# apache/cassandra

Hardware: NVIDIA H100
Metric: compaction MB/s (uncompressed in) (higher is better)
Workload: dtype u8

## Files before the change

cassandra_b200/csrc/compact.cu:

```cuda
#include "engine.cuh"
#include "scan.cuh"
#include "codec_defs.cuh"
#include "partition.cuh"
#include "partition_tile.cuh"
#include "meta.cuh"
#include "index_walk.cuh"
#include <climits>
#include <vector>
#include <algorithm>
#include <cmath>

using namespace b200c;

namespace b200c {

int compress_stream_device(b200c_ctx* c, int comp, const uint8_t* d_in, uint64_t n, int chunk_len, int max_clen,
                           uint8_t* d_out, uint64_t out_cap, uint64_t* d_offs, uint64_t* out_len, uint32_t* digest, int ws_base);
int compress_slots_device(b200c_ctx* c, int comp, const uint8_t* d_in, uint64_t n, int chunk_len, int max_clen,
                          uint8_t* slots, int stride, uint32_t* file_len, uint32_t* seg_raw);
int pack_digest_device(b200c_ctx* c, const uint8_t* slots, int stride, const uint32_t* file_len, const uint32_t* seg_raw, uint64_t nchunks,
                       uint8_t* d_out, uint64_t out_cap, uint64_t* d_offs, uint64_t* out_len, uint32_t* digest, int ws_base);
int decompress_stream_device(b200c_ctx* c, int comp, const uint8_t* d_data, uint64_t data_len, const uint64_t* d_offs, uint64_t nchunks,
                             int chunk_len, int max_clen, uint64_t data_length, uint8_t* d_out, int verify, ChunkErr* d_err, uint64_t chunk0, uint64_t count, int tag,
                             const uint8_t* tail, uint64_t tail_off);
int decompress_multi_device(b200c_ctx* c, K1Seg* segs, int nseg, int verify, ChunkErr* d_err, int ws_slot);
int raw_chunks_device(b200c_ctx* c, bool ingest, const RawArgs& a);
int raw_stream_device(b200c_ctx* c, const uint8_t* d_in, uint64_t n, int chunk_len, uint8_t* d_out, uint64_t* d_crc, uint32_t* digest, int ws_base);

enum { IB = 256 };
static_assert(IW_PAD <= 64, "the Index.db workspace keeps 64 bytes behind every input (index_walk.cuh)");
#ifndef B200C_K4_STAGED_DEFAULT
#define B200C_K4_STAGED_DEFAULT 0
#endif
#ifndef B200C_K1_BATCH_DEFAULT
#define B200C_K1_BATCH_DEFAULT true
#endif
#define NONE64 (~0ull)

enum { WS_U = 16, WS_CD, WS_CO, WS_IDX, WS_PARAMS, WS_BBASE, WS_ISTART, WS_ICNT, WS_IEND, WS_IHIT, WS_IBAD, WS_ISCAN,
// ... 511 lines not shown
    return ((uint64_t)fanin_class(m, bound, wide_bound) * ntiles + (j >> tile_shift)) * SORT_BINS + (m - 1) * SORT_BUCKETS + bucket;
}
__global__ void __launch_bounds__(256) k_class_hist(const uint64_t* __restrict__ op_first, const uint64_t* __restrict__ bound, uint64_t nparts,
                                                    uint32_t tile_shift, uint64_t ntiles, uint64_t wide_bound, unsigned long long* __restrict__ hist) {
    for (uint64_t j = (uint64_t)blockIdx.x * blockDim.x + threadIdx.x; j < nparts; j += (uint64_t)gridDim.x * blockDim.x)
        atomicAdd(&hist[sort_key((uint32_t)(op_first[j + 1] - op_first[j]), bound[j], j, tile_shift, ntiles, wide_bound)], 1ull);
}
__global__ void __launch_bounds__(256) k_fanin_scatter(const uint64_t* __restrict__ op_first, const uint64_t* __restrict__ bound, uint64_t nparts,
                                                       uint32_t tile_shift, uint64_t ntiles, uint64_t wide_bound, unsigned long long* __restrict__ cursor, uint32_t* __restrict__ list) {
    uint64_t j = (uint64_t)blockIdx.x * blockDim.x + threadIdx.x;
    bool valid = j < nparts;
    uint64_t key = valid ? sort_key((uint32_t)(op_first[j + 1] - op_first[j]), bound[j], j, tile_shift, ntiles, wide_bound) : ~0ull;
    uint32_t peers = __match_any_sync(FULL_MASK, key);
    int lane = threadIdx.x & 31, leader = __ffs(peers) - 1;
    unsigned long long base = 0;
    if (valid && lane == leader) base = atomicAdd(&cursor[key], (unsigned long long)__popc(peers));
    base = __shfl_sync(FULL_MASK, base, leader);
    if (valid) list[base + __popc(peers & ((1u << lane) - 1u))] = (uint32_t)j;
}

typedef Cur32 K4Cur;
enum { SLOT_BYTES = sizeof(K4Cur), K4_SMEM_COLS = 8 };

struct K4Args {
    const CParams* P; const uint64_t* contrib; const uint64_t* op_first; const uint32_t* list; const uint64_t* upos; const uint64_t* pbase;
    const uint64_t* kp; const uint16_t* klen; const int64_t* tok;
    uint64_t* dsize; uint32_t* ipay; uint32_t* nblk; uint32_t* ihead; uint32_t* st_munf; uint32_t* st_rows; uint8_t* ovf;
    const uint64_t* doff; const uint64_t* dcapv; const uint64_t* dpos; const uint64_t* ipos; uint8_t* dbase; uint8_t* iout; DevErr* err; int mode;
    uint64_t jlo, jhi;
    const uint64_t* ioff; const uint32_t* icapv; uint8_t* iscr;
    int m3_nblk;
    const uint8_t* only_big;
    StatGlobal* sg; TdropTable* td; uint32_t* ccount;
};

template <bool EMIT> __device__ __forceinline__ bool k4_prologue(const K4Args& a, uint64_t j, uint8_t*& dout, uint64_t& dcap, uint64_t& dposv, uint8_t*& iout, uint32_t& nbf, uint32_t& ipf, uint32_t& ixs_cap) {
    dout = nullptr; dcap = ~0ull; dposv = 0; iout = nullptr; nbf = 0; ipf = 0; ixs_cap = 0;
    if (!EMIT) return true;
    if (a.mode == 1) {
        if (a.only_big && !a.only_big[j]) return false;
        dout = a.dbase + a.doff[j]; dcap = a.dcapv[j];
        uint32_t slot = a.icapv[j];
        if (slot) { iout = a.iscr + a.ioff[j]; nbf = (slot - IXS_HEAD) / IXS_BLOCK_STRIDE; ixs_cap = nbf * IXS_PER_BLOCK; }
        return true;
    }
    if (!a.dsize[j] || j < a.jlo || j >= a.jhi) return false;
    if (a.mode == 3 && !(a.ovf[j] || (a.m3_nblk && a.nblk[j] > 1))) return false;
    dout = a.dbase + a.dpos[j]; dposv = a.dpos[j]; iout = a.iout + a.ipos[j]; nbf = a.nblk[j]; ipf = a.ipay[j];
    return true;
}
template <bool EMIT> __device__ __forceinline__ void k4_epilogue(const K4Args& a, uint64_t j, uint64_t c0, PartOut out, PartStats st, int e) {
    if (EMIT && a.mode >= 2) { if (e || out.dsize != a.dsize[j]) report_err(a.err, 8, 0, j); return; }
    if (e) { uint64_t en = a.contrib[c0]; int src = (int)((en >> 56) & 0x7F); report_err(a.err, e == PERR_UNSUPPORTED ? 9 : 4, src, a.upos[a.pbase[src] + (en & 0xFFFFFFFFFFull)] - a.P->in[src].ubase); out = PartOut{0, 0, 0, 0, 0}; st = PartStats{0, 0}; }
    a.dsize[j] = out.dsize; a.ipay[j] = out.ipay; a.nblk[j] = out.nblk; a.ihead[j] = out.ihead; a.ovf[j] = (uint8_t)out.ovf;
    if (a.ccount) a.ccount[j] = out.cells;
    a.st_munf[j] = (uint32_t)st.merged_unfiltereds; a.st_rows[j] = (uint32_t)st.rows_out;
}

template <int M_CAP, int NT, bool EMIT, bool CX = false>
__global__ void __launch_bounds__(NT, 384 / NT) k_partition_thr(const K4Args a, uint64_t lo, uint64_t hi) {
    extern __shared__ __align__(16) uint8_t s_raw[];
    const int ncols_s = a.P->mcols <= K4_SMEM_COLS ? a.P->mcols : 0;
    const int stride = M_CAP * SLOT_BYTES + ncols_s * (int)sizeof(MCell) + 8;
    K4Cur* cur = (K4Cur*)(s_raw + (size_t)threadIdx.x * stride);
    MCell merged_local[MAXCOLS];
    MCell* merged = ncols_s ? (MCell*)(cur + M_CAP) : merged_local;
    DT open_dt[M_CAP];
    uint64_t t = lo + (uint64_t)blockIdx.x * NT + threadIdx.x;
    if (t >= hi) return;
    uint64_t j = a.list[t];
    uint8_t *dout, *iout; uint64_t dcap, dposv; uint32_t nbf, ipf, ixs_cap;
    if (!k4_prologue<EMIT>(a, j, dout, dcap, dposv, iout, nbf, ipf, ixs_cap)) return;
    uint64_t c0 = a.op_first[j]; uint32_t m = (uint32_t)(a.op_first[j + 1] - c0);
    PartOut out{0, 0, 0, 0, 0}; PartStats st{0, 0}; int e = 0;
    StatAcc acc; const bool stats = a.sg != nullptr && a.mode == 1;
    if (stats) acc.init(a.P->now, a.td);
    if (m > (uint32_t)M_CAP) e = PERR_UNSUPPORTED;
    else process_partition<EMIT, K4Cur, XlateGlobal, M_CAP, CX>(*a.P, XlateGlobal(), a.contrib, c0, m, a.upos, a.pbase, a.kp, a.klen, a.tok, dout, dcap, dposv, iout, nbf, ipf, ixs_cap, cur, open_dt, merged, out, st, e, stats ? &acc : nullptr);
    k4_epilogue<EMIT>(a, j, c0, out, st, e);
    if (stats && !e) stat_flush(a.sg, acc);
}

template <int S, bool EMIT>
__global__ void __launch_bounds__(128) k_partition_warp(const K4Args a, uint64_t lo, uint64_t hi) {
    extern __shared__ __align__(16) uint8_t s_raw[];
    auto tile = cg::tiled_partition<32>(cg::this_thread_block());
    const int tid = threadIdx.x / 32;
// ... 102 lines not shown
    StatAcc acc; acc.init(sP->now, a.td);
    for (uint32_t t = tid; t < np; t += ST_THREADS) {
        const uint32_t j = j0 + s_order[t];
        const uint64_t cj = a.op_first[j]; const uint32_t m = (uint32_t)(a.op_first[j + 1] - cj);
        const uint32_t m_uni = min((uint32_t)ST_MAXM, __reduce_max_sync(__activemask(), m));
        uint8_t *dout, *iout; uint64_t dcap, dposv; uint32_t nbf, ipf, ixs_cap;
        if (!k4_prologue<true>(a, j, dout, dcap, dposv, iout, nbf, ipf, ixs_cap)) continue;
        PartOut out{0, 0, 0, 0, 0}; PartStats st{0, 0}; int e = 0;
        if (m > (uint32_t)ST_MAXM || cj - c0 + m > (uint64_t)ST_CUR_CAP) e = PERR_UNSUPPORTED;
        else process_partition<true>(*sP, xl, a.contrib, cj, m, a.upos, a.pbase, a.kp, a.klen, a.tok, dout, dcap, dposv, iout, nbf, ipf, ixs_cap, curs + (cj - c0), open_dt, merged, out, st, e,
                                     a.sg ? &acc : nullptr, m_uni);
        k4_epilogue<true>(a, j, cj, out, st, e);
    }
    if (a.sg) stat_flush_warp(a.sg, acc);
}

__global__ void __launch_bounds__(256) k_bounds(const uint64_t* __restrict__ contrib, const uint64_t* __restrict__ op_first, uint64_t nparts,
                                                const uint64_t* __restrict__ upos, const uint64_t* __restrict__ pbase, uint64_t* __restrict__ bound,
                                                uint32_t column_index_size, uint32_t* __restrict__ icap, uint32_t* __restrict__ insz, uint8_t* __restrict__ big) {
    uint64_t j = (uint64_t)blockIdx.x * blockDim.x + threadIdx.x;
    if (j >= nparts) return;
    uint64_t sum = 0;
    for (uint64_t c = op_first[j]; c < op_first[j + 1]; c++) { uint64_t e = contrib[c]; uint64_t g = pbase[(e >> 56) & 0x7F] + (e & 0xFFFFFFFFFFull); sum += upos[g + 1] - upos[g]; }
    uint64_t b = (sum + (sum >> 2) + 32 + 15) & ~15ull;
    bound[j] = b;
    insz[j] = (uint32_t)min(sum, (uint64_t)0xFFFFFFFFull);
    big[j] = (sum > (uint64_t)ST_MAXP || op_first[j + 1] - op_first[j] > (uint64_t)ST_MAXM) ? 1 : 0;
    uint64_t nb_max = b / column_index_size + 2;
    icap[j] = (b > column_index_size && nb_max < (1u << 23)) ? (uint32_t)(IXS_HEAD + nb_max * IXS_BLOCK_STRIDE) : 0u;
}

__global__ void __launch_bounds__(256) k_gather(uint64_t nparts, const uint64_t* __restrict__ dsize, const uint64_t* __restrict__ dpos, const uint64_t* __restrict__ bpos,
                                                const uint8_t* __restrict__ ovf, const uint8_t* __restrict__ scratch, uint8_t* __restrict__ uout) {
    uint64_t j = (uint64_t)blockIdx.x * 8 + (threadIdx.x >> 5);
    if (j >= nparts) return;
    uint64_t n = dsize[j];
    if (!n || ovf[j]) return;
    const uint8_t* s = scratch + bpos[j]; uint8_t* d = uout + dpos[j];
    int lane = threadIdx.x & 31;
    for (uint64_t i = lane; i < n; i += 32) d[i] = s[i];
}

__global__ void __launch_bounds__(256) k_index_simple(const CParams* __restrict__ Pp, uint64_t nparts, const uint64_t* __restrict__ contrib, const uint64_t* __restrict__ op_first,
        const uint64_t* __restrict__ upos, const uint64_t* __restrict__ pbase, const uint64_t* __restrict__ dsize, const uint64_t* __restrict__ dpos,
        const uint32_t* __restrict__ nblk, const uint8_t* __restrict__ ovf, const uint32_t* __restrict__ ihead, const uint64_t* __restrict__ ipos, uint8_t* __restrict__ iout) {
    uint64_t j = (uint64_t)blockIdx.x * blockDim.x + threadIdx.x;
    if (j >= nparts || !dsize[j] || nblk[j] > 1 || ovf[j]) return;
    uint64_t e = contrib[op_first[j]]; uint64_t g = pbase[(e >> 56) & 0x7F] + (e & 0xFFFFFFFFFFull);
    const uint8_t* k = Pp->U + upos[g];
    uint32_t n = ihead[j];
    Sink<true> s{iout + ipos[j], 0, true, ~0ull};
    s.copy(k, n); s.vint(dpos[j]); s.u8(0);
}

__global__ void __launch_bounds__(128) k_index_promoted(const CParams* __restrict__ Pp, uint64_t nparts, const uint64_t* __restrict__ contrib, const uint64_t* __restrict__ op_first,
        const uint64_t* __restrict__ upos, const uint64_t* __restrict__ pbase, const uint64_t* __restrict__ dsize, const uint64_t* __restrict__ dpos,
        const uint32_t* __restrict__ nblk, const uint8_t* __restrict__ ovf, const uint32_t* __restrict__ ihead, const uint32_t* __restrict__ ipay, const uint64_t* __restrict__ ipos,
        const uint64_t* __restrict__ ioff, const uint32_t* __restrict__ icap, const uint8_t* __restrict__ iscr, uint8_t* __restrict__ iout) {
    uint64_t j = (uint64_t)blockIdx.x * blockDim.x + threadIdx.x;
    if (j >= nparts || !dsize[j] || nblk[j] <= 1 || ovf[j]) return;
    uint64_t e = contrib[op_first[j]]; uint64_t g = pbase[(e >> 56) & 0x7F] + (e & 0xFFFFFFFFFFull);
    const uint8_t* k = Pp->U + upos[g];
    const uint8_t* slot = iscr + ioff[j];
    const uint32_t nb_max = (icap[j] - IXS_HEAD) / IXS_BLOCK_STRIDE, nb = nblk[j], n = ihead[j];
    DT pd; pd.mfda = ((const int64_t*)slot)[0]; pd.ldt = ((const int64_t*)slot)[1];
    const uint32_t pdsz = dt_is_live(pd) ? 1u : 12u, hdr_len = (uint32_t)((const int64_t*)slot)[2];
    const uint32_t infos = ipay[j] - vint_size(hdr_len) - pdsz - vint_size(nb) - 4 * nb;
    Sink<true> s{iout + ipos[j], 0, true, ~0ull};
    s.copy(k, n); s.vint(dpos[j]); s.vint(ipay[j]);
    s.vint(hdr_len); write_partition_dt(s, pd); s.vint(nb);
    s.copy(slot + IXS_HEAD + 4 * (size_t)nb_max, infos); s.copy(slot + IXS_HEAD, 4 * nb);
}

// ... 63 lines not shown
template <bool WIDE> int k4_staged(b200c_ctx* c, const K4Args& ka, uint64_t ntiles, size_t smem, const uint32_t* tstart, const uint8_t* big) {
    B200C_LAUNCH(c, k_partition_staged<WIDE>, (unsigned)ntiles, ST_THREADS, smem, ka, tstart, big);
    return B200C_OK;
}
template <bool WIDE> void k4_staged_attr(size_t smem) { cudaFuncSetAttribute(k_partition_staged<WIDE>, cudaFuncAttributeMaxDynamicSharedMemorySize, (int)smem); }

struct CompactCall {
    b200c_ctx* const c; const b200c_manifest* const m; b200c_result* const res;
    const bool dev, lcs; const int K;
    const bool raw_out, to_host_stream;
    const cudaMemcpyKind in_kind;
    Pinned* const P; const cudaStream_t st, cs;
    const std::chrono::steady_clock::time_point t_start = std::chrono::steady_clock::now();
    bool want_meta = false, two_pass = false;
    int rc = B200C_OK;

    struct Need { uint64_t h2d_a, h2d_b, k1_a, k1_b; };
    bool have_summaries = true, sliced = false, deferred = false, istream = false;
    int nr = 1;
    std::vector<IdxSlice> isl;
    std::vector<int64_t> T;
    std::vector<std::vector<IdxSlice>> psl;
    std::vector<uint64_t> pustart;
    std::vector<std::vector<uint64_t>> psb;
    std::vector<Need> need;
    std::vector<uint64_t> range_bytes, range_end;
    std::vector<uint64_t> h2d_next, k1_next;
    std::vector<std::vector<uint64_t>> co_host;
    std::vector<uint64_t> ubase, ibase, cbase, obase, bbase;
    uint64_t uo = 0, io = 0, co = 0, oo = 0, in_bytes = 0, bytes_read = 0;
    CParams hp; std::vector<InDesc> hin;

    uint8_t *U = nullptr, *CD = nullptr, *IDX = nullptr; uint64_t *CO = nullptr, *d_bbase = nullptr, *d_summ = nullptr; CParams* dP = nullptr;
    DevErr* d_err = nullptr; ChunkErr* d_cerr = nullptr; RunStats* d_stats = nullptr; unsigned long long *d_hist = nullptr, *d_rbytes = nullptr;
    std::vector<const uint8_t*> k1_data, k1_tail; std::vector<const uint64_t*> k1_offs; std::vector<uint64_t> k1_tail_off; std::vector<K1Seg> segs;
    int k1_batch_env = 0;
    StatGlobal* d_sg = nullptr; TdropTable* d_td = nullptr; uint32_t* d_bloom = nullptr; uint8_t *d_mkeys = nullptr, *d_sument = nullptr; uint64_t* d_sumoff = nullptr;
    uint64_t written_total = 0, samples_total = 0, sument_bound = 0, bloom_words = 0; uint32_t meta_interval = 128;
    uint64_t total_parts = 0, slow_inputs = 0; std::vector<uint64_t> pcount, pbase;
    int64_t* d_tok = nullptr; uint64_t *d_kp = nullptr, *d_upos = nullptr, *d_pbase = nullptr, *d_pcount = nullptr, *d_range = nullptr; uint16_t* d_klen = nullptr;
    OutStream os; uint64_t L = 0;
    uint64_t ubase_total = 0, ilen_total = 0, ncontrib_total = 0, nparts_total = 0;
    uint64_t tail_len = 0; const uint8_t* tail_ptr = nullptr;
    bool index_fits = true;
    uint64_t nparts = 0, ulen_out = 0, ilen_out = 0, n_le8 = 0, n_le12 = 0, n_le16 = 0, n_le32 = 0;
    uint64_t *d_contrib = nullptr, *d_opfirst = nullptr, *d_bound = nullptr, *d_bpos = nullptr, *d_ioff = nullptr, *d_dsize = nullptr, *d_dpos = nullptr, *d_ipos = nullptr, *d_wrank = nullptr;
    uint32_t *d_list = nullptr, *d_icap = nullptr, *d_insz = nullptr, *d_ipay = nullptr, *d_nblk = nullptr, *d_ihead = nullptr, *d_isize = nullptr;
    uint32_t *d_stmunf = nullptr, *d_strows = nullptr, *d_ccount = nullptr, *d_wflag = nullptr; uint8_t *d_ovf = nullptr, *d_big = nullptr;
    uint8_t *UOUT = nullptr, *IOUT = nullptr, *ISCR = nullptr, *SCRATCH = nullptr;
    size_t smem8 = 0, smem12 = 0, smem16 = 0, smem64 = 0, cell_smem32 = 0;
    K4Args ka;
    int lcs_stride = 0; uint8_t* slots = nullptr; uint32_t *file_len = nullptr, *seg_raw = nullptr; uint64_t *woffs = nullptr, *d_cut = nullptr;
    struct Mark { int stage; cudaEvent_t ev; };
    std::vector<Mark> marks;

    CompactCall(b200c_ctx* c_, const b200c_manifest* m_, b200c_result* res_, int flags)
        : c(c_), m(m_), res(res_), dev((flags & B200C_FLAG_DEVICE_PTRS) != 0), lcs(m_->max_sstable_bytes != 0), K(m_->ninputs),
          raw_out(m_->out_compressor == COMP_UNCOMPRESSED), to_host_stream(!dev && !lcs), in_kind(dev ? cudaMemcpyDeviceToDevice : cudaMemcpyHostToDevice),
          P(c_->h_pinned), st(c_->stream), cs(c_->copy_stream) {
        cudaSetDevice(c->device);
        c->prog_stage.store(0); c->prog_scanned.store(0);
        for (int i = 0; i < B200C_MAX_INPUTS; i++) c->prog_input_pos[i].store(0);
        c->prog_seq.fetch_add(1);
    }
    ~CompactCall() {
        if (c->timing) timing_end(c);
        cudaStreamSynchronize(st); cudaStreamSynchronize(cs); cudaStreamSynchronize(c->copy_out);
// ... 184 lines not shown
        }
        T = t2; psl = p2; pustart = u2;
        return true;
    }

    int workspace() {
        B200C_TRY(ws_typed(c, WS_U, uo + 64, &U));
        k1_data.assign(K, nullptr); k1_tail.assign(K, nullptr); k1_offs.assign(K, nullptr); k1_tail_off.assign(K, ~0ull);
        if (dev) {
            std::vector<uint64_t> tb(K + 1, 0);
            auto tail_window = [](const b200c_input& in) -> uint64_t { return in.compressor == COMP_UNCOMPRESSED ? 0 : std::min(in.data_len, k1_tail_window(chunk_max_compressed(in.compressor, in.chunk_len), in.chunk_len)); };
            for (int i = 0; i < K; i++) tb[i + 1] = tb[i] + ((tail_window(m->inputs[i]) + 64 + 15) & ~15ull);
            uint8_t* TAIL; B200C_TRY(ws_typed(c, WS_K1TAIL, tb[K] + 64, &TAIL));
            for (int i = 0; i < K; i++) {
                const b200c_input& in = m->inputs[i];
                const uint64_t win = tail_window(in);
                k1_data[i] = in.data; k1_offs[i] = in.chunk_offsets; k1_tail[i] = TAIL + tb[i]; k1_tail_off[i] = in.data_len - win;
                if (win) B200C_CUDA_TRY(c, cudaMemcpyAsync(TAIL + tb[i], in.data + (in.data_len - win), win, cudaMemcpyDeviceToDevice, st));
            }
        } else {
            B200C_TRY(ws_typed(c, WS_CD, co + 64, &CD));
            B200C_TRY(ws_typed(c, WS_CO, oo + 1, &CO));
            for (int i = 0; i < K; i++) { k1_data[i] = m->inputs[i].compressor == COMP_UNCOMPRESSED ? U + ubase[i] : CD + cbase[i]; k1_offs[i] = CO + obase[i]; }
        }
        B200C_TRY(ws_typed(c, WS_IDX, io + 64, &IDX));
        psb.assign(nr, std::vector<uint64_t>(K + 1, 0));
        uint64_t summ_total = 0;
        for (int r = 0; r < nr; r++) for (int i = 0; i <= K; i++) { psb[r][i] = summ_total; if (i < K) summ_total += psl[r][i].s_count; }
        B200C_TRY(ws_typed(c, WS_SUMM, summ_total + 1, &d_summ));
        { uint8_t* pp; B200C_TRY(ws_typed(c, WS_PARAMS, sizeof(CParams) + sizeof(InDesc) * (size_t)K, &pp)); dP = (CParams*)pp; hp.in = (const InDesc*)(pp + sizeof(CParams)); }
        B200C_TRY(ws_typed(c, WS_BBASE, (size_t)K + 1, &d_bbase));
        { uint8_t* p; B200C_TRY(ws_typed(c, WS_ERR2, 4096, &p)); d_err = (DevErr*)p; d_cerr = (ChunkErr*)(p + 64); d_stats = (RunStats*)(p + 128); d_hist = (unsigned long long*)(p + 256); }
        d_rbytes = (unsigned long long*)(d_stats + 1) + 1;
        hp.U = U;
        if (m->npurge_ranges) {
            int64_t* d_pt; B200C_TRY(ws_typed(c, WS_PURGE, 2 * (size_t)m->npurge_ranges, &d_pt));
            B200C_CUDA_TRY(c, cudaMemcpyAsync(d_pt, m->purge_range_hi, 8 * (size_t)m->npurge_ranges, cudaMemcpyHostToDevice, st));
            B200C_CUDA_TRY(c, cudaMemcpyAsync(d_pt + m->npurge_ranges, m->purge_range_max_ts, 8 * (size_t)m->npurge_ranges, cudaMemcpyHostToDevice, st));
            hp.purge_hi = d_pt; hp.purge_ts = d_pt + m->npurge_ranges; hp.npurge = m->npurge_ranges;
        }
        meta_interval = m->min_index_interval > 0 ? (uint32_t)m->min_index_interval : 128u;
        bloom_words = (want_meta && res->outputs[0].filter) ? m->bloom_words : 0;
        if (want_meta) {
            B200C_TRY(ws_typed(c, WS_META_SG, 1, &d_sg));
            B200C_TRY(ws_typed(c, WS_META_TD, 1, &d_td));
            B200C_TRY(ws_typed(c, WS_META_BLOOM, bloom_words * 2 + 16, &d_bloom));
            B200C_TRY(ws_typed(c, WS_META_KEYS, (size_t)2 * 65536, &d_mkeys));
            std::vector<uint8_t> init(sizeof(StatGlobal), 0); StatGlobal* g0 = (StatGlobal*)init.data();
            g0->min_ts = I64_MAX; g0->max_ts = I64_MIN; g0->min_ldt = I64_MAX; g0->max_ldt = I64_MIN; g0->min_ttl = INT_MAX; g0->max_ttl = INT_MIN;
            auto offsets = [](long long* o, int n) { long long last = 1; o[0] = 1; for (int i = 1; i < n; i++) { long long next = llround((double)last * 1.2); if (next == last) next++; o[i] = next; last = next; } };
            offsets(g0->psize_off, META_PSIZE - 1); offsets(g0->cells_off, META_CELLS - 1);
            B200C_CUDA_TRY(c, cudaMemcpyAsync(d_sg, init.data(), sizeof(StatGlobal), cudaMemcpyHostToDevice, st));
            B200C_CUDA_TRY(c, cudaStreamSynchronize(st));
            B200C_CUDA_TRY(c, cudaMemsetAsync(d_td, 0, sizeof(TdropTable), st));
            B200C_CUDA_TRY(c, cudaMemsetAsync(d_td->key, 0xFF, sizeof(d_td->key), st));
            if (bloom_words) B200C_CUDA_TRY(c, cudaMemsetAsync(d_bloom, 0, bloom_words * 8, st));
        }
        B200C_CUDA_TRY(c, cudaMemsetAsync(d_err, 0xFF, 64, st));
        B200C_CUDA_TRY(c, cudaMemsetAsync(d_cerr, 0xFF, 64, st));
        B200C_CUDA_TRY(c, cudaMemsetAsync(d_stats, 0, 128 + MAXK * 8 + 128, st));
        B200C_CUDA_TRY(c, cudaMemcpyAsync((void*)hp.in, hin.data(), sizeof(InDesc) * (size_t)K, cudaMemcpyHostToDevice, st));
        B200C_CUDA_TRY(c, cudaMemcpyAsync(dP, &hp, sizeof(hp), cudaMemcpyHostToDevice, st));
        B200C_CUDA_TRY(c, cudaMemcpyAsync(d_bbase, bbase.data(), (K + 1) * 8, cudaMemcpyHostToDevice, st));
        return B200C_OK;
    }

// ... 359 lines not shown
        if (hp.ncx || hp.ctr_mask || hp.sctr_mask) {
            if (!emit) { c->err = "B200C_K4_TWO_PASS with multi-cell columns"; return B200C_EUNSUPPORTED; }
            B200C_TRY((k4_thr<8, 128, true>(c, ka, true, 0, n_le8, smem8)));
            B200C_TRY((k4_thr<12, 64, true>(c, ka, true, n_le8, n_le12, smem12)));
            B200C_TRY((k4_thr<16, 64, true>(c, ka, true, n_le12, n_le16, smem16)));
            return k4_thr<64, 32, true>(c, ka, true, n_le16, nparts, smem64);
        }
        B200C_TRY((k4_thr<8, 128>(c, ka, emit, 0, n_le8, smem8)));
        B200C_TRY((k4_thr<12, 64>(c, ka, emit, n_le8, n_le12, smem12)));
        B200C_TRY((k4_thr<16, 64>(c, ka, emit, n_le12, n_le16, smem16)));
        B200C_TRY(k4_warp<1>(c, ka, emit, n_le16, n_le32, cell_smem32));
        return k4_warp<2>(c, ka, emit, n_le32, nparts, cell_smem32);
    }
    int k4() {
        mark(3);
        c->prog_stage.store(4);
        B200C_TRY(ws_typed(c, WS_DSIZE, nparts + 1, &d_dsize));
        B200C_TRY(ws_typed(c, WS_DPOS, nparts + 2, &d_dpos));
        B200C_TRY(ws_typed(c, WS_IPOS, nparts + 2, &d_ipos));
        B200C_TRY(ws_typed(c, WS_IPAY, nparts + 1, &d_ipay));
        B200C_TRY(ws_typed(c, WS_NBLK, nparts + 1, &d_nblk));
        B200C_TRY(ws_typed(c, WS_IHEAD, nparts + 1, &d_ihead));
        B200C_TRY(ws_typed(c, WS_ISIZE, nparts + 1, &d_isize));
        B200C_TRY(ws_typed(c, WS_STMUNF, nparts + 1, &d_stmunf));
        B200C_TRY(ws_typed(c, WS_STROWS, nparts + 1, &d_strows));
        B200C_TRY(ws_typed(c, WS_OVF, nparts + 1, &d_ovf));
        const size_t cols_s = hp.mcols <= K4_SMEM_COLS ? (size_t)hp.mcols * sizeof(MCell) : 0;
        smem8 = (size_t)128 * (8 * SLOT_BYTES + cols_s + 8); smem12 = (size_t)64 * (12 * SLOT_BYTES + cols_s + 8); smem16 = (size_t)64 * (16 * SLOT_BYTES + cols_s + 8);
        smem64 = (size_t)32 * (64 * SLOT_BYTES + cols_s + 8); cell_smem32 = (size_t)4 * hp.mcols * sizeof(MCell);
        memset(&ka, 0, sizeof(ka));
        ka.P = dP; ka.contrib = d_contrib; ka.op_first = d_opfirst; ka.list = d_list; ka.upos = d_upos; ka.pbase = d_pbase; ka.kp = d_kp; ka.klen = d_klen; ka.tok = d_tok;
        ka.dsize = d_dsize; ka.ipay = d_ipay; ka.nblk = d_nblk; ka.ihead = d_ihead; ka.st_munf = d_stmunf; ka.st_rows = d_strows; ka.ovf = d_ovf;
        ka.dpos = d_dpos; ka.ipos = d_ipos; ka.err = d_err; ka.jlo = 0; ka.jhi = nparts; ka.m3_nblk = two_pass ? 1 : 0;
        if (want_meta) {
            B200C_TRY(ws_typed(c, WS_CCOUNT, nparts + 1, &d_ccount));
            B200C_TRY(ws_typed(c, WS_META_FLAG, nparts + 1, &d_wflag));
            B200C_TRY(ws_typed(c, WS_META_WRANK, nparts + 2, &d_wrank));
            ka.sg = d_sg; ka.td = d_td; ka.ccount = d_ccount;
        }
        if (c->k4_attr_set != (int)(smem8 + 1)) {
            const char* carveout = getenv("B200C_K4_CARVEOUT");
            k4_attr<8, 128, true>(smem8, carveout); k4_attr<8, 128, false>(smem8); k4_attr<8, 128, true, true>(smem8);
            k4_attr<12, 64, true>(smem12, carveout); k4_attr<12, 64, false>(smem12); k4_attr<12, 64, true, true>(smem12);
            k4_attr<16, 64, true>(smem16, carveout); k4_attr<16, 64, false>(smem16); k4_attr<16, 64, true, true>(smem16);
            k4_attr<64, 32, true, true>(smem64);
            c->k4_attr_set = (int)(smem8 + 1);
        }
        ulen_out = 0; ilen_out = 0;
        if (!nparts) return B200C_OK;
        if (two_pass) {
            B200C_CUDA_TRY(c, cudaMemsetAsync(d_ovf, 0, nparts, st));
            B200C_TRY(launch_k4(0));
        } else B200C_TRY(k4_scratch());
        B200C_LAUNCH(c, k_sum_stats, 8 * c->nsm, 256, 0, nparts, d_dsize, d_stmunf, d_strows, d_stats);
        B200C_TRY(exclusive_scan<uint64_t>(c, d_dsize, nparts, d_dpos, WS_SCANA, 0));
        if (ubase_total) B200C_LAUNCH(c, k_add_u64, (unsigned)((nparts + 1 + 255) / 256), 256, 0, d_dpos, nparts + 1, ubase_total);
        B200C_LAUNCH(c, k_index_sizes, (unsigned)((nparts + 255) / 256), 256, 0, nparts, d_dsize, d_dpos, d_ipay, d_ihead, d_isize);
        B200C_TRY(exclusive_scan<uint32_t>(c, d_isize, nparts, d_ipos, WS_SCANA + 3, 0));
        B200C_CUDA_TRY(c, cudaMemcpyAsync(&P->data_end, d_dpos + nparts, 8, cudaMemcpyDeviceToHost, st));
        B200C_CUDA_TRY(c, cudaMemcpyAsync(&P->index_len, d_ipos + nparts, 8, cudaMemcpyDeviceToHost, st));
        B200C_CUDA_TRY(c, cudaMemcpyAsync(&P->err, d_err, 8, cudaMemcpyDeviceToHost, st));
        if (want_meta) {
            B200C_LAUNCH(c, k_written_flags, (unsigned)((nparts + 255) / 256), 256, 0, nparts, d_dsize, d_wflag);
            B200C_TRY(exclusive_scan<uint32_t>(c, d_wflag, nparts, d_wrank, WS_SCANA, 0));
            B200C_CUDA_TRY(c, cudaMemcpyAsync(&P->written, d_wrank + nparts, 8, cudaMemcpyDeviceToHost, st));
        }
        B200C_CUDA_TRY(c, cudaStreamSynchronize(st));
        if (P->err != ~0ull) {
            const int in = (int)((P->err >> 48) & 0xFF); const uint64_t off = P->err & 0xFFFFFFFFFFFFull;
            if ((int)(P->err >> 56) == 9) { corrupt(in, 4, 0, off, ""); c->err = "unsupported feature in input " + std::to_string(in) + " (outside the envelope: shadowable deletion, a fan-in or layout the kernels refuse, or a counter context the reference never writes inside a merge)"; return B200C_EUNSUPPORTED; }
            return corrupt(in, 4, 0, off, "malformed Data.db in input " + std::to_string(in) + " near offset " + std::to_string(off));
        }
        ulen_out = P->data_end - ubase_total; ilen_out = P->index_len;
        return B200C_OK;
    }
    int k4_scratch() {
        B200C_TRY(exclusive_scan<uint64_t>(c, d_bound, nparts, d_bpos, WS_SCANA, 0));
        B200C_TRY(exclusive_scan<uint32_t>(c, d_icap, nparts, d_ioff, WS_SCANA + 3, 0));
        B200C_CUDA_TRY(c, cudaMemcpyAsync(&P->scratch_len, d_bpos + nparts, 8, cudaMemcpyDeviceToHost, st));
        B200C_CUDA_TRY(c, cudaMemcpyAsync(&P->iscr_len, d_ioff + nparts, 8, cudaMemcpyDeviceToHost, st));
        B200C_CUDA_TRY(c, cudaStreamSynchronize(st));
        B200C_TRY(ws_typed(c, WS_SCRATCH, P->scratch_len + 64, &SCRATCH));
        B200C_TRY(ws_typed(c, WS_ISCR, P->iscr_len + 64, &ISCR));
        ka.doff = d_bpos; ka.dcapv = d_bound; ka.dbase = SCRATCH; ka.iout = nullptr; ka.ioff = d_ioff; ka.icapv = d_icap; ka.iscr = ISCR;
        const bool staged = !hp.ncx && !hp.ctr_mask && !hp.sctr_mask && []() { const char* e = getenv("B200C_K4_STAGED"); return e ? atoi(e) != 0 : (B200C_K4_STAGED_DEFAULT != 0); }();
        if (!staged) return launch_k4(1);
        uint64_t *d_inpos, *d_tscan; uint32_t *d_mark, *d_tstart; unsigned long long* d_nbig = (unsigned long long*)(d_stats + 1);
        B200C_TRY(ws_typed(c, WS_INPOS, nparts + 2, &d_inpos));
        B200C_TRY(ws_typed(c, WS_TMARK, nparts + 2, &d_mark));
        B200C_TRY(ws_typed(c, WS_TSCAN, nparts + 2, &d_tscan));
        B200C_TRY(ws_typed(c, WS_TSTART, nparts + 2, &d_tstart));
        B200C_TRY(exclusive_scan<uint32_t>(c, d_insz, nparts, d_inpos, WS_SCANA, 0));
        B200C_CUDA_TRY(c, cudaMemsetAsync(d_nbig, 0, 8, st));
        B200C_LAUNCH(c, k_tile_marks, (unsigned)((nparts + 255) / 256), 256, 0, nparts, d_inpos, d_opfirst, d_big, d_mark, d_nbig);
        B200C_TRY(exclusive_scan<uint32_t>(c, d_mark, nparts, d_tscan, WS_SCANA, 0));
        B200C_LAUNCH(c, k_tile_starts, (unsigned)((nparts + 1 + 255) / 256), 256, 0, nparts, d_mark, d_tscan, d_tstart);
        B200C_CUDA_TRY(c, cudaMemcpyAsync(&P->ntiles, d_tscan + nparts, 8, cudaMemcpyDeviceToHost, st));
        B200C_CUDA_TRY(c, cudaMemcpyAsync(&P->nbig, d_nbig, 8, cudaMemcpyDeviceToHost, st));
        B200C_CUDA_TRY(c, cudaStreamSynchronize(st));
        const bool wide = m->ncolumns > K4_SMEM_COLS;
        const size_t smem_st = (size_t)ST_HEAD + ST_STAGE_CAP + (size_t)ST_CUR_CAP * sizeof(CurS) + (wide ? 0 : (size_t)ST_THREADS * hp.mcols * sizeof(MCell)) + 16;
        if (c->k4s_attr_set != (int)smem_st) { k4_staged_attr<false>(smem_st); k4_staged_attr<true>(smem_st); c->k4s_attr_set = (int)smem_st; }
        ka.mode = 1; ka.only_big = nullptr;
        B200C_TRY(wide ? k4_staged<true>(c, ka, P->ntiles, smem_st, d_tstart, d_big) : k4_staged<false>(c, ka, P->ntiles, smem_st, d_tstart, d_big));
        if (P->nbig) { ka.only_big = d_big; B200C_TRY(launch_k4(1)); ka.only_big = nullptr; }
        return B200C_OK;
    }
    int emit(int r) {
        mark(4);
        if (raw_out && to_host_stream && r >= 2) B200C_CUDA_TRY(c, cudaStreamWaitEvent(st, c->ev_pool[EV_UOUT_FREE + (r & 1)], 0));
        B200C_TRY(ws_typed(c, (r & 1) ? WS_UOUT2 : WS_UOUT, tail_len + ulen_out + 64, &UOUT));
        if (r) B200C_CUDA_TRY(c, cudaStreamWaitEvent(st, c->ev_pool[EV_INDEX_FREE], 0));
        B200C_TRY(ws_typed(c, WS_IOUT, ilen_out + 64, &IOUT));
        if (tail_len) B200C_CUDA_TRY(c, cudaMemcpyAsync(UOUT, tail_ptr, tail_len, cudaMemcpyDeviceToDevice, st));
        uint8_t* const ubias = (uint8_t*)((uintptr_t)UOUT + tail_len - ubase_total);
        if (!nparts || !ulen_out) return B200C_OK;
        ka.dbase = ubias; ka.iout = IOUT; ka.doff = nullptr; ka.dcapv = nullptr;
        if (two_pass) return launch_k4(2);
        B200C_LAUNCH(c, k_gather, (unsigned)((nparts + 7) / 8), 256, 0, nparts, d_dsize, d_dpos, d_bpos, d_ovf, SCRATCH, ubias);
        B200C_LAUNCH(c, k_index_simple, (unsigned)((nparts + 255) / 256), 256, 0, dP, nparts, d_contrib, d_opfirst, d_upos, d_pbase, d_dsize, d_dpos, d_nblk, d_ovf, d_ihead, d_ipos, IOUT);
        B200C_LAUNCH(c, k_index_promoted, (unsigned)((nparts + 127) / 128), 128, 0, dP, nparts, d_contrib, d_opfirst, d_upos, d_pbase, d_dsize, d_dpos, d_nblk, d_ovf, d_ihead, d_ipay, d_ipos,
                     d_ioff, d_icap, ISCR, IOUT);
        return launch_k4(3);
    }
    int meta() {
        const uint64_t ns = (written_total + P->written + meta_interval - 1) / meta_interval - (written_total + meta_interval - 1) / meta_interval;
        uint32_t *d_samplej, *d_esize; uint64_t* d_epos;
        B200C_TRY(ws_typed(c, WS_META_SAMPLE, ns + 1, &d_samplej));
        B200C_TRY(ws_typed(c, WS_META_ESIZE, ns + 1, &d_esize));
        B200C_TRY(ws_typed(c, WS_META_EPOS, ns + 2, &d_epos));
        MetaArgs ma; memset(&ma, 0, sizeof(ma));
        ma.P = dP; ma.contrib = d_contrib; ma.op_first = d_opfirst; ma.upos = d_upos; ma.pbase = d_pbase; ma.dsize = d_dsize; ma.ipos = d_ipos; ma.ihead = d_ihead;
        ma.ccount = d_ccount; ma.wrank = d_wrank; ma.nparts = nparts; ma.index_base = ilen_total; ma.written_base = written_total; ma.sg = d_sg;
        ma.bloom = d_bloom; ma.bloom_bits = bloom_words * 64; ma.bloom_k = m->bloom_hash_count; ma.interval = meta_interval; ma.sample_j = d_samplej;
        ma.first_key = d_mkeys; ma.last_key = d_mkeys + 65536;
        B200C_LAUNCH(c, k_meta_keys, (unsigned)((nparts + 255) / 256), 256, 0, ma);
        if (ns && res->outputs[0].summary) {
            B200C_LAUNCH(c, k_summary_sizes, (unsigned)((ns + 255) / 256), 256, 0, ma, ns, d_esize);
            B200C_TRY(exclusive_scan<uint32_t>(c, d_esize, ns, d_epos, WS_SCANA, 0));
            B200C_CUDA_TRY(c, cudaMemcpyAsync(&P->summary_len, d_epos + ns, 8, cudaMemcpyDeviceToHost, st));
            B200C_CUDA_TRY(c, cudaStreamSynchronize(st));
            B200C_TRY(ws_grow_keep<uint8_t>(c, WS_META_SUMENT, sument_bound + P->summary_len + 64, sument_bound, &d_sument));
            B200C_TRY(ws_grow_keep<uint64_t>(c, WS_META_SUMOFF, samples_total + ns + 2, samples_total, &d_sumoff));
            B200C_LAUNCH(c, k_summary_emit, (unsigned)((ns + 255) / 256), 256, 0, ma, ns, d_epos, d_sument, d_sumoff);
            B200C_LAUNCH(c, k_meta_advance, 1, 1, 0, d_sg, ns, d_epos);
            sument_bound += P->summary_len; samples_total += ns;
        }
        written_total += P->written;
        return B200C_OK;
    }
    int k5_stream(int r) {
        mark(5);
        c->prog_stage.store(5);
        if (!to_host_stream) return B200C_OK;
        b200c_output& out0 = res->outputs[0];
        if (ilen_out) {
// ... 177 lines not shown
        B200C_TRY(ws_typed(c, WS_LCS4, ilen_out + 64, &IOUTF));
        B200C_TRY(ws_typed(c, WS_OOFFS, nch_total + 4, &d_ooffs));
        const uint64_t file_bound = b200c_compress_bound(comp, ulen_out, (int)L);
        if (!raw_out) B200C_TRY(ws_typed(c, WS_DOUT, file_bound + 64, &d_dout));
        res->required_data_cap = res->required_index_cap = res->required_chunk_cap = 0;
        uint64_t jlo = 0, start_b = 0; int f = 0;
        double est_ratio = 0.5;
        if (!raw_out) { uint64_t ci = 0, ui = 0; for (int i = 0; i < K; i++) { ci += m->inputs[i].data_len; ui += m->inputs[i].data_length; } if (ui) est_ratio = std::min(1.0, std::max(0.05, (double)ci / (double)ui)); }
        while (jlo < nparts && start_b < ulen_out) {
            B200C_TRY(check_cancel());
            uint64_t jhi, done;
            B200C_TRY(lcs_cut(jlo, start_b, est_ratio, jhi, done));
            uint64_t end_b = ulen_out;
            if (jhi < nparts) { B200C_CUDA_TRY(c, cudaMemcpyAsync(&P->file_end, d_dpos + jhi, 8, cudaMemcpyDeviceToHost, st)); B200C_CUDA_TRY(c, cudaStreamSynchronize(st)); end_b = P->file_end; }
            const uint64_t flen = end_b - start_b, fchunks = (flen + L - 1) / L, nfull = flen / L, tail = flen % L;
            uint64_t out_len = 0; uint32_t digest = 0;
            if (raw_out) { B200C_TRY(raw_stream_device(c, UOUT + start_b, flen, (int)L, nullptr, d_ooffs, &digest, WS_CODEC)); out_len = flen; }
            else {
                if (tail && !(end_b == ulen_out && done == (ulen_out - start_b + L - 1) / L))
                    B200C_TRY(compress_slots_device(c, comp, UOUT + start_b + nfull * L, tail, (int)L, m->out_max_compressed_len, slots + nfull * lcs_stride, lcs_stride, file_len + nfull, seg_raw + nfull));
                B200C_TRY(pack_digest_device(c, slots, lcs_stride, file_len, seg_raw, fchunks, d_dout, file_bound, d_ooffs, &out_len, &digest, WS_CODEC));
            }
            const uint64_t cnt = jhi - jlo;
            B200C_LAUNCH(c, k_rel_pos, (unsigned)((cnt + 1 + 255) / 256), 256, 0, d_dpos, jlo, jhi, start_b, d_dposf);
            B200C_LAUNCH(c, k_index_sizes, (unsigned)((cnt + 255) / 256), 256, 0, cnt, d_dsize + jlo, d_dposf + jlo, d_ipay + jlo, d_ihead + jlo, d_isize + jlo);
            B200C_TRY(exclusive_scan<uint32_t>(c, d_isize + jlo, cnt, d_iposf + jlo, WS_SCANA + 3, 0));
            B200C_CUDA_TRY(c, cudaMemsetAsync(d_fstats, 0, sizeof(RunStats), st));
            B200C_LAUNCH(c, k_sum_stats, 2 * c->nsm, 256, 0, cnt, d_dsize + jlo, d_stmunf + jlo, d_strows + jlo, d_fstats);
            B200C_LAUNCH(c, k_index_simple, (unsigned)((cnt + 255) / 256), 256, 0, dP, cnt, d_contrib, d_opfirst + jlo, d_upos, d_pbase, d_dsize + jlo, d_dposf + jlo,
                         d_nblk + jlo, d_ovf + jlo, d_ihead + jlo, d_iposf + jlo, IOUTF);
            if (!two_pass) B200C_LAUNCH(c, k_index_promoted, (unsigned)((cnt + 127) / 128), 128, 0, dP, cnt, d_contrib, d_opfirst + jlo, d_upos, d_pbase, d_dsize + jlo, d_dposf + jlo,
                                        d_nblk + jlo, d_ovf + jlo, d_ihead + jlo, d_ipay + jlo, d_iposf + jlo, d_ioff + jlo, d_icap + jlo, ISCR, IOUTF);
            ka.dbase = UOUT + start_b; ka.iout = IOUTF; ka.dpos = d_dposf; ka.ipos = d_iposf; ka.jlo = jlo; ka.jhi = jhi;
            B200C_TRY(launch_k4(3));
            B200C_CUDA_TRY(c, cudaMemcpyAsync(&P->file_index_len, d_iposf + jhi, 8, cudaMemcpyDeviceToHost, st));
            B200C_CUDA_TRY(c, cudaMemcpyAsync(P->file_stats, d_fstats, sizeof(RunStats), cudaMemcpyDeviceToHost, st));
            B200C_CUDA_TRY(c, cudaStreamSynchronize(st));
            FileOut fo{out_len, P->file_index_len, fchunks, flen, digest, {}}; memcpy(&fo.rs, P->file_stats, sizeof(fo.rs));
            if (flen && out_len) est_ratio = std::min(1.0, std::max(0.05, (double)out_len / (double)flen));
            res->required_data_cap = std::max<uint64_t>(res->required_data_cap, out_len);
            res->required_index_cap = std::max<uint64_t>(res->required_index_cap, fo.index_len);
            res->required_chunk_cap = std::max<uint64_t>(res->required_chunk_cap, fchunks);
            if (fo.rs.partitions_out) {
                if (f >= res->noutputs_cap) { c->err = "more output files than output slots"; rc = B200C_ETOOSMALL; }
                else {
                    bool sent;
                    B200C_TRY(publish(res->outputs[f], fo, true, raw_out ? UOUT + start_b : d_dout, IOUTF, d_ooffs, dev ? cudaMemcpyDeviceToDevice : cudaMemcpyDeviceToHost, &sent));
                    if (sent) describe(res->outputs[f], fo);
                }
                f++;
            }
            jlo = jhi; start_b = end_b;
        }
        RunStats rs; B200C_TRY(finish_common(rs));
        res->noutputs = f;
        return B200C_OK;
    }
};

}

extern "C" {

int b200c_compact(b200c_ctx* c, const b200c_manifest* m, b200c_result* res, int flags) {
    if (!c || !m || !res) return B200C_EINVAL;
    CompactCall call(c, m, res, flags);
    B200C_TRY(call.validate());
// ... 36 lines not shown
```

cassandra_b200/csrc/engine.cuh:

```cuda
#pragma once
#include <cstdio>
#include <cstring>
#include <string>
#include <atomic>
#include <chrono>
#include <vector>
#include "../../include/b200c.h"
#include "common.cuh"

namespace b200c {

enum { WS_SLOTS = 160, WS_K5_ENT = 150, WS_K1_REC = 151, WS_K1_NSEQ = 152 };

struct WsBuf { void* p = nullptr; size_t cap = 0; };

enum { MAX_RANGES = 16 };
enum { EV_OUT_PIECE = 0, EV_RANGE = 200, EV_INDEX_FREE = 220, EV_INDEX_READY = 221, EV_UOUT_FREE = 230, EV_POOL = 256 };
struct Pinned;

}

struct b200c_ctx {
    int device = 0;
    int nsm = 0;
// ... 80 lines not shown
}

struct OutStream {
    enum { MAX_PIECES = 96 };
    b200c_ctx* c = nullptr; int comp = 0, L = 0, max_clen = 0, stride = 0, ws_base = 0;
    uint8_t* h_out = nullptr; uint64_t h_cap = 0;
    uint32_t *file_len = nullptr, *seg_raw = nullptr, *acc = nullptr; uint64_t *d_offs = nullptr, *bases = nullptr;
    uint8_t* img[2] = {nullptr, nullptr}; uint64_t img_cap[2] = {0, 0};
    uint64_t nchunks = 0, ulen = 0, copied = 0; int piece = 0; bool fits = true;
    bool raw = false; uint64_t* ends = nullptr;
};
int out_stream_begin(OutStream& o, b200c_ctx* c, int comp, int chunk_len, int max_clen, uint8_t* h_out, uint64_t h_cap, int ws_base);
int out_stream_append(OutStream& o, const uint8_t* d_in, uint64_t nbytes);
int out_stream_finish(OutStream& o, uint64_t* out_len, uint32_t* digest, uint64_t** d_offs_out);

static_assert(EV_OUT_PIECE + 2 * OutStream::MAX_PIECES <= EV_RANGE && EV_RANGE + MAX_RANGES <= EV_INDEX_FREE &&
              EV_INDEX_FREE < EV_INDEX_READY && EV_INDEX_READY < EV_UOUT_FREE && EV_UOUT_FREE + 2 <= EV_POOL, "ev_pool slots overlap");

struct Pinned {
    uint64_t packed_len;
    uint32_t digest;
    uint64_t chunk_err;
    uint64_t os_end[OutStream::MAX_PIECES];
    uint32_t os_digest;
    uint64_t cerr, err;
    uint64_t range[2 * B200C_MAX_INPUTS];
    uint64_t scan[B200C_MAX_INPUTS + 1];
    uint32_t bad[B200C_MAX_INPUTS + 1];
    uint64_t plan[2 * MAX_RANGES * B200C_MAX_INPUTS];
    uint64_t nparts, class_end[4];
    uint64_t scratch_len, iscr_len;
    uint64_t ntiles, nbig;
    uint64_t data_end, index_len, written;
    uint64_t summary_len;
    uint64_t run_stats[3], hist[B200C_MAX_INPUTS], bytes_in_range;
    uint64_t cut[2], file_end, file_index_len, file_stats[3];
};
enum { H_PINNED_CAP = 1 << 16 };
static_assert(sizeof(Pinned) <= H_PINNED_CAP, "b200c_ctx::h_pinned");

template <typename TIn> int exclusive_scan(b200c_ctx* c, const TIn* in, uint64_t n, uint64_t* out, int scan_slot0, int depth = 0);

}
```

Before: 35820.

## Vectorize partition gather with warp-cooperative 16-byte copies and skip empty overflow pass

The gather kernel used to copy one partition per warp a byte at a time. It now assigns 32 partitions to each warp, prefix-scans their 16-byte output words, and spreads aligned vector loads and funnel-shifted stores across lanes, so small partitions no longer leave most lanes idle and the copy moves wide words instead of bytes. Separately, a device counter of overflowed partitions is copied back to the host, and the mode-3 partition relaunch is skipped when that count is zero. The cost is extra shuffle and address arithmetic per word, plus one atomic per overflowed partition. The skip depends on the counter being reset between runs; the diff does not show where that happens.

```diff
diff --git a/cassandra_b200/csrc/compact.cu b/cassandra_b200/csrc/compact.cu
--- a/cassandra_b200/csrc/compact.cu
+++ b/cassandra_b200/csrc/compact.cu
@@ -5,6 +5,7 @@
 #include "partition_tile.cuh"
 #include "meta.cuh"
 #include "index_walk.cuh"
+#include "gather.cuh"
 #include <climits>
 #include <vector>
 #include <algorithm>
@@ -582,6 +583,7 @@
     int m3_nblk;
     const uint8_t* only_big;
     StatGlobal* sg; TdropTable* td; uint32_t* ccount;
+    unsigned long long* novf;
 };
 
 template <bool EMIT> __device__ __forceinline__ bool k4_prologue(const K4Args& a, uint64_t j, uint8_t*& dout, uint64_t& dcap, uint64_t& dposv, uint8_t*& iout, uint32_t& nbf, uint32_t& ipf, uint32_t& ixs_cap) {
@@ -603,6 +605,7 @@
     if (EMIT && a.mode >= 2) { if (e || out.dsize != a.dsize[j]) report_err(a.err, 8, 0, j); return; }
     if (e) { uint64_t en = a.contrib[c0]; int src = (int)((en >> 56) & 0x7F); report_err(a.err, e == PERR_UNSUPPORTED ? 9 : 4, src, a.upos[a.pbase[src] + (en & 0xFFFFFFFFFFull)] - a.P->in[src].ubase); out = PartOut{0, 0, 0, 0, 0}; st = PartStats{0, 0}; }
     a.dsize[j] = out.dsize; a.ipay[j] = out.ipay; a.nblk[j] = out.nblk; a.ihead[j] = out.ihead; a.ovf[j] = (uint8_t)out.ovf;
+    if (out.ovf && a.novf) atomicAdd(a.novf, 1ull);
     if (a.ccount) a.ccount[j] = out.cells;
     a.st_munf[j] = (uint32_t)st.merged_unfiltereds; a.st_rows[j] = (uint32_t)st.rows_out;
 }
@@ -771,13 +774,9 @@
 
 __global__ void __launch_bounds__(256) k_gather(uint64_t nparts, const uint64_t* __restrict__ dsize, const uint64_t* __restrict__ dpos, const uint64_t* __restrict__ bpos,
                                                 const uint8_t* __restrict__ ovf, const uint8_t* __restrict__ scratch, uint8_t* __restrict__ uout) {
-    uint64_t j = (uint64_t)blockIdx.x * 8 + (threadIdx.x >> 5);
-    if (j >= nparts) return;
-    uint64_t n = dsize[j];
-    if (!n || ovf[j]) return;
-    const uint8_t* s = scratch + bpos[j]; uint8_t* d = uout + dpos[j];
-    int lane = threadIdx.x & 31;
-    for (uint64_t i = lane; i < n; i += 32) d[i] = s[i];
+    const uint64_t j0 = ((uint64_t)blockIdx.x * 8 + (threadIdx.x >> 5)) * 32;
+    if (j0 >= nparts) return;
+    gather_warp(j0, nparts, dsize, dpos, bpos, ovf, scratch, uout, (int)(threadIdx.x & 31));
 }
 
 __global__ void __launch_bounds__(256) k_index_simple(const CParams* __restrict__ Pp, uint64_t nparts, const uint64_t* __restrict__ contrib, const uint64_t* __restrict__ op_first,
@@ -907,7 +906,7 @@
     CParams hp; std::vector<InDesc> hin;
 
     uint8_t *U = nullptr, *CD = nullptr, *IDX = nullptr; uint64_t *CO = nullptr, *d_bbase = nullptr, *d_summ = nullptr; CParams* dP = nullptr;
-    DevErr* d_err = nullptr; ChunkErr* d_cerr = nullptr; RunStats* d_stats = nullptr; unsigned long long *d_hist = nullptr, *d_rbytes = nullptr;
+    DevErr* d_err = nullptr; ChunkErr* d_cerr = nullptr; RunStats* d_stats = nullptr; unsigned long long *d_hist = nullptr, *d_rbytes = nullptr, *d_novf = nullptr;
     std::vector<const uint8_t*> k1_data, k1_tail; std::vector<const uint64_t*> k1_offs; std::vector<uint64_t> k1_tail_off; std::vector<K1Seg> segs;
     int k1_batch_env = 0;
     StatGlobal* d_sg = nullptr; TdropTable* d_td = nullptr; uint32_t* d_bloom = nullptr; uint8_t *d_mkeys = nullptr, *d_sument = nullptr; uint64_t* d_sumoff = nullptr;
@@ -1158,6 +1157,7 @@
         B200C_TRY(ws_typed(c, WS_BBASE, (size_t)K + 1, &d_bbase));
         { uint8_t* p; B200C_TRY(ws_typed(c, WS_ERR2, 4096, &p)); d_err = (DevErr*)p; d_cerr = (ChunkErr*)(p + 64); d_stats = (RunStats*)(p + 128); d_hist = (unsigned long long*)(p + 256); }
         d_rbytes = (unsigned long long*)(d_stats + 1) + 1;
+        d_novf = d_rbytes + 1;
         hp.U = U;
         if (m->npurge_ranges) {
             int64_t* d_pt; B200C_TRY(ws_typed(c, WS_PURGE, 2 * (size_t)m->npurge_ranges, &d_pt));
@@ -1583,6 +1583,7 @@
         ka.P = dP; ka.contrib = d_contrib; ka.op_first = d_opfirst; ka.list = d_list; ka.upos = d_upos; ka.pbase = d_pbase; ka.kp = d_kp; ka.klen = d_klen; ka.tok = d_tok;
         ka.dsize = d_dsize; ka.ipay = d_ipay; ka.nblk = d_nblk; ka.ihead = d_ihead; ka.st_munf = d_stmunf; ka.st_rows = d_strows; ka.ovf = d_ovf;
         ka.dpos = d_dpos; ka.ipos = d_ipos; ka.err = d_err; ka.jlo = 0; ka.jhi = nparts; ka.m3_nblk = two_pass ? 1 : 0;
+        ka.novf = d_novf;
         if (want_meta) {
             B200C_TRY(ws_typed(c, WS_CCOUNT, nparts + 1, &d_ccount));
             B200C_TRY(ws_typed(c, WS_META_FLAG, nparts + 1, &d_wflag));
@@ -1611,6 +1612,7 @@
         B200C_CUDA_TRY(c, cudaMemcpyAsync(&P->data_end, d_dpos + nparts, 8, cudaMemcpyDeviceToHost, st));
         B200C_CUDA_TRY(c, cudaMemcpyAsync(&P->index_len, d_ipos + nparts, 8, cudaMemcpyDeviceToHost, st));
         B200C_CUDA_TRY(c, cudaMemcpyAsync(&P->err, d_err, 8, cudaMemcpyDeviceToHost, st));
+        B200C_CUDA_TRY(c, cudaMemcpyAsync(&P->novf, d_novf, 8, cudaMemcpyDeviceToHost, st));
         if (want_meta) {
             B200C_LAUNCH(c, k_written_flags, (unsigned)((nparts + 255) / 256), 256, 0, nparts, d_dsize, d_wflag);
             B200C_TRY(exclusive_scan<uint32_t>(c, d_wflag, nparts, d_wrank, WS_SCANA, 0));
@@ -1668,11 +1670,11 @@
         if (!nparts || !ulen_out) return B200C_OK;
         ka.dbase = ubias; ka.iout = IOUT; ka.doff = nullptr; ka.dcapv = nullptr;
         if (two_pass) return launch_k4(2);
-        B200C_LAUNCH(c, k_gather, (unsigned)((nparts + 7) / 8), 256, 0, nparts, d_dsize, d_dpos, d_bpos, d_ovf, SCRATCH, ubias);
+        B200C_LAUNCH(c, k_gather, (unsigned)((nparts + 255) / 256), 256, 0, nparts, d_dsize, d_dpos, d_bpos, d_ovf, SCRATCH, ubias);
         B200C_LAUNCH(c, k_index_simple, (unsigned)((nparts + 255) / 256), 256, 0, dP, nparts, d_contrib, d_opfirst, d_upos, d_pbase, d_dsize, d_dpos, d_nblk, d_ovf, d_ihead, d_ipos, IOUT);
         B200C_LAUNCH(c, k_index_promoted, (unsigned)((nparts + 127) / 128), 128, 0, dP, nparts, d_contrib, d_opfirst, d_upos, d_pbase, d_dsize, d_dpos, d_nblk, d_ovf, d_ihead, d_ipay, d_ipos,
                      d_ioff, d_icap, ISCR, IOUT);
-        return launch_k4(3);
+        return P->novf ? launch_k4(3) : B200C_OK;
     }
     int meta() {
         const uint64_t ns = (written_total + P->written + meta_interval - 1) / meta_interval - (written_total + meta_interval - 1) / meta_interval;
@@ -1916,7 +1918,7 @@
             if (!two_pass) B200C_LAUNCH(c, k_index_promoted, (unsigned)((cnt + 127) / 128), 128, 0, dP, cnt, d_contrib, d_opfirst + jlo, d_upos, d_pbase, d_dsize + jlo, d_dposf + jlo,
                                         d_nblk + jlo, d_ovf + jlo, d_ihead + jlo, d_ipay + jlo, d_iposf + jlo, d_ioff + jlo, d_icap + jlo, ISCR, IOUTF);
             ka.dbase = UOUT + start_b; ka.iout = IOUTF; ka.dpos = d_dposf; ka.ipos = d_iposf; ka.jlo = jlo; ka.jhi = jhi;
-            B200C_TRY(launch_k4(3));
+            if (two_pass || P->novf) B200C_TRY(launch_k4(3));
             B200C_CUDA_TRY(c, cudaMemcpyAsync(&P->file_index_len, d_iposf + jhi, 8, cudaMemcpyDeviceToHost, st));
             B200C_CUDA_TRY(c, cudaMemcpyAsync(P->file_stats, d_fstats, sizeof(RunStats), cudaMemcpyDeviceToHost, st));
             B200C_CUDA_TRY(c, cudaStreamSynchronize(st));
diff --git a/cassandra_b200/csrc/engine.cuh b/cassandra_b200/csrc/engine.cuh
--- a/cassandra_b200/csrc/engine.cuh
+++ b/cassandra_b200/csrc/engine.cuh
@@ -136,6 +136,7 @@
     uint64_t scratch_len, iscr_len;
     uint64_t ntiles, nbig;
     uint64_t data_end, index_len, written;
+    uint64_t novf;
     uint64_t summary_len;
     uint64_t run_stats[3], hist[B200C_MAX_INPUTS], bytes_in_range;
     uint64_t cut[2], file_end, file_index_len, file_stats[3];
diff --git a/cassandra_b200/csrc/gather.cuh b/cassandra_b200/csrc/gather.cuh
--- /dev/null
+++ b/cassandra_b200/csrc/gather.cuh
@@ -0,0 +1,84 @@
+#pragma once
+#include <cstdint>
+#include <cuda_runtime.h>
+
+namespace b200c {
+
+enum { GATHER_UNROLL = 4 };
+constexpr unsigned GATHER_ALL = 0xFFFFFFFFu;
+
+struct GatherPart { uintptr_t dst, src; uint64_t n; };
+
+struct GatherWord { uintptr_t D; uint32_t b0, b1; uint32_t r[4]; };
+__device__ __forceinline__ GatherWord gather_load(const GatherPart& p, uint64_t k) {
+    GatherWord g;
+    const uintptr_t D = (p.dst & ~(uintptr_t)15) + 16 * (uintptr_t)k;
+    const uintptr_t lo = D > p.dst ? D : p.dst, hi = D + 16 < p.dst + p.n ? D + 16 : p.dst + p.n;
+    const uintptr_t S = p.src + (D - p.dst);
+    const uintptr_t slo = p.src + (lo - p.dst), shi = p.src + (hi - p.dst);
+    const uintptr_t A0 = S & ~(uintptr_t)15, A1 = A0 + 16;
+    uint4 w0 = make_uint4(0, 0, 0, 0), w1 = w0;
+    if (A0 + 16 > slo) w0 = __ldg((const uint4*)A0);
+    if (A1 < shi) w1 = __ldg((const uint4*)A1);
+    uint32_t a[8] = {w0.x, w0.y, w0.z, w0.w, w1.x, w1.y, w1.z, w1.w};
+    const uint32_t o = (uint32_t)(S & 15), sh = 8 * (o & 3);
+    if (o & 8) {
+#pragma unroll
+        for (int i = 0; i < 6; i++) a[i] = a[i + 2];
+    }
+    if (o & 4) {
+#pragma unroll
+        for (int i = 0; i < 5; i++) a[i] = a[i + 1];
+    }
+#pragma unroll
+    for (int i = 0; i < 4; i++) g.r[i] = __funnelshift_r(a[i], a[i + 1], sh);
+    g.D = D; g.b0 = (uint32_t)(lo - D); g.b1 = (uint32_t)(hi - D);
+    return g;
+}
+__device__ __forceinline__ void gather_store(const GatherWord& g) {
+    if (g.b0 == 0 && g.b1 == 16) { *(uint4*)g.D = make_uint4(g.r[0], g.r[1], g.r[2], g.r[3]); return; }
+#pragma unroll
+    for (uint32_t i = 0; i < 4; i++) {
+        if (g.b0 <= 4 * i && 4 * i + 4 <= g.b1) { ((uint32_t*)g.D)[i] = g.r[i]; continue; }
+#pragma unroll
+        for (uint32_t b = 0; b < 4; b++) if (g.b0 <= 4 * i + b && 4 * i + b < g.b1) ((uint8_t*)g.D)[4 * i + b] = (uint8_t)(g.r[i] >> (8 * b));
+    }
+}
+
+__device__ __forceinline__ void gather_warp(uint64_t j0, uint64_t nparts, const uint64_t* __restrict__ dsize, const uint64_t* __restrict__ dpos,
+                                            const uint64_t* __restrict__ bpos, const uint8_t* __restrict__ ovf, const uint8_t* __restrict__ scratch,
+                                            uint8_t* __restrict__ uout, int lane) {
+    const uint64_t j = j0 + (uint64_t)lane;
+    GatherPart mine{0, 0, 0};
+    uint32_t nw = 0;
+    if (j < nparts) {
+        const uint64_t n = dsize[j];
+        if (n && !ovf[j]) {
+            mine.dst = (uintptr_t)(uout + dpos[j]); mine.src = (uintptr_t)(scratch + bpos[j]); mine.n = n;
+            nw = (uint32_t)((((mine.dst + n - 1) & ~(uintptr_t)15) - (mine.dst & ~(uintptr_t)15)) / 16 + 1);
+        }
+    }
+    uint32_t incl = nw;
+#pragma unroll
+    for (int d = 1; d < 32; d <<= 1) { const uint32_t v = __shfl_sync(GATHER_ALL, incl, (lane - d) & 31); if (lane >= d) incl += v; }
+    const uint32_t total = __shfl_sync(GATHER_ALL, incl, 31);
+    for (uint32_t base = 0; base < total; base += 32 * GATHER_UNROLL) {
+        GatherWord g[GATHER_UNROLL]; bool on[GATHER_UNROLL];
+#pragma unroll
+        for (int u = 0; u < GATHER_UNROLL; u++) {
+            const uint32_t w = base + 32 * u + (uint32_t)lane;
+            uint32_t q = 0;
+#pragma unroll
+            for (uint32_t s = 16; s; s >>= 1) if (__shfl_sync(GATHER_ALL, incl, (int)(q + s - 1)) <= w) q += s;
+            GatherPart p;
+            p.dst = __shfl_sync(GATHER_ALL, mine.dst, (int)q); p.src = __shfl_sync(GATHER_ALL, mine.src, (int)q); p.n = __shfl_sync(GATHER_ALL, mine.n, (int)q);
+            const uint32_t first = __shfl_sync(GATHER_ALL, incl - nw, (int)q);
+            on[u] = w < total;
+            if (on[u]) g[u] = gather_load(p, w - first);
+        }
+#pragma unroll
+        for (int u = 0; u < GATHER_UNROLL; u++) if (on[u]) gather_store(g[u]);
+    }
+}
+
+}
```

After: 36450, median of 6. 1.02x the previous value.
